# ToyotaResearchInstitute/conex

Measured on AMD Instinct MI355X. Metric: Newton KKT-solves/sec (assemble+factor+solve), 1000x(20x20) PSD blocks, fp64, higher is better.
Workload: dtype f64

## Files before the change

### conex_amd/csrc/dense_elim.hip.h

```cpp
#pragma once
#include "device_utils.h"

namespace cxk {

__device__ __forceinline__ void SqrtAndInverse(double d, double& root, double& inv) {
  const double r0 = __builtin_amdgcn_rsq(d);
  double g = d * r0, h = 0.5 * r0;
  double e = fma(-h, g, 0.5);
  g = fma(g, e, g);
  h = fma(h, e, h);
  e = fma(-h, g, 0.5);
  g = fma(g, e, g);
  h = fma(h, e, h);
  const double res = fma(-g, g, d);
  root = fma(res, h, g);
  inv = h + h;
}

template <int LEN, int C0, int C1, int BASE>
struct DppColumns {
  static __device__ __forceinline__ void run(double (&a)[LEN], double w, double v) {
    if constexpr (C0 < C1) {
      asm("v_fmac_f64_dpp %0, %1, %2 row_newbcast:%3 row_mask:0xf bank_mask:0xf"
          : "+v"(a[C0])
          : "v"(w), "v"(v), "n"(C0 - BASE));
      DppColumns<LEN, C0 + 1, C1, BASE>::run(a, w, v);
    }
  }
};

__device__ __forceinline__ void DppOperandFence(double& x, double& y, double& z) {
  asm("s_nop 1" : "+v"(x), "+v"(y), "+v"(z));
}

__device__ __forceinline__ double EvenRowsToOddRows(double v) {
  typedef unsigned u2 __attribute__((ext_vector_type(2)));
  const unsigned lo = __double2loint(v), hi = __double2hiint(v);
  const u2 a = __builtin_amdgcn_permlane16_swap(lo, lo, false, false);
  const u2 b = __builtin_amdgcn_permlane16_swap(hi, hi, false, false);
  return __hiloint2double(b.x, a.x);
}

template <int NSMAX, int SMAX, int J, int NRHS = 1, bool CHECK = true>
struct ElimSteps {
  static constexpr int LEN = NSMAX + SMAX + NRHS, RB = NSMAX + SMAX;
  static __device__ __forceinline__ void run(double (&a)[LEN], int lane, bool& bad, int ns) {
    if constexpr (J == 0 && NSMAX > 0) {
      const double d = ReadLane(a[0], 0);
      if constexpr (CHECK) bad |= !(d > 0.0);
      double root, inv;
      SqrtAndInverse(d, root, inv);
      step(a, lane, bad, root, inv, ns);
    }
  }
  static __device__ __forceinline__ void step(double (&a)[LEN], int lane, bool& bad, double root, double inv, int ns) {
    if constexpr (J < NSMAX) {
      if (J >= ns) return;
      a[J] = (lane == J) ? root : a[J] * inv;
      double root1 = 1.0, inv1 = 1.0;
      auto next_pivot = [&]() {
        if constexpr (J + 1 < NSMAX) {
          const double d1 = ReadLane(a[J + 1], J + 1);
          if constexpr (CHECK) bad |= !(d1 > 0.0);
          SqrtAndInverse(d1, root1, inv1);
        }
      };
      if constexpr (NSMAX + SMAX <= 16) {
        double naj = -a[J];
        double dummy = 0.0;
        DppOperandFence(dummy, naj, a[J]);
        DppColumns<LEN, J + 1, (J + 2 < NSMAX + SMAX ? J + 2 : NSMAX + SMAX), 0>::run(a, a[J], naj);
        next_pivot();
        DppColumns<LEN, J + 2, NSMAX + SMAX, 0>::run(a, a[J], naj);
      } else if constexpr (NSMAX + SMAX <= 32 && NSMAX != 16) {
        const RowPair xp = Swap16(a[J]);
        double x0 = xp.a, x1 = xp.b;
        double naj = -a[J];
        DppOperandFence(x0, x1, naj);
        constexpr int kEnd = NSMAX + SMAX;
        constexpr int n1 = (J + 2 < kEnd) ? J + 2 : kEnd;
        if constexpr (J + 1 < 16)
          DppColumns<LEN, J + 1, (n1 < 16 ? n1 : 16), 0>::run(a, x0, naj);
        else
          DppColumns<LEN, J + 1, n1, 16>::run(a, x1, naj);
        next_pivot();
        constexpr int kLo0 = (J + 2 < 16) ? J + 2 : 16, kLo1 = (kEnd < 16) ? kEnd : 16;
        constexpr int kHi0 = (J + 2 > 16) ? J + 2 : 16;
        DppColumns<LEN, kLo0, kLo1, 0>::run(a, x0, naj);
        DppColumns<LEN, kHi0, kEnd, 16>::run(a, x1, naj);
      } else if constexpr (NSMAX == 16 && SMAX <= 16) {
        double x = EvenRowsToOddRows(a[J]);
        double naj = -a[J];
        DppOperandFence(x, naj, a[J]);
        DppColumns<LEN, J + 1, (J + 2 < NSMAX ? J + 2 : NSMAX), 0>::run(a, x, naj);
        next_pivot();
        DppColumns<LEN, J + 2, NSMAX, 0>::run(a, x, naj);
        DppColumns<LEN, NSMAX, NSMAX + SMAX, NSMAX>::run(a, a[J], naj);
      } else {
        if constexpr (J + 1 < NSMAX + SMAX) a[J + 1] = fma(-ReadLane(a[J], J + 1), a[J], a[J + 1]);
        next_pivot();
#pragma unroll
        for (int c = J + 2; c < NSMAX + SMAX; c++) a[c] = fma(-ReadLane(a[J], c), a[J], a[c]);
      }
#pragma unroll
      for (int q = 0; q < NRHS; q++) {
        const double yj = ReadLane(a[RB + q], J) * inv;
        if (lane > J)
          a[RB + q] = fma(-yj, a[J], a[RB + q]);
        else if (lane == J)
          a[RB + q] = yj;
      }
      ElimSteps<NSMAX, SMAX, J + 1, NRHS, CHECK>::step(a, lane, bad, root1, inv1, ns);
    }
  }
};

}
```

### conex_amd/csrc/kkt_context.hip

```cpp
#include "kkt_launch.h"
#include "kernels_gemm.hip.h"

namespace cxk_host {

int Fail(cxk_context* ctx, const char* msg) {
  ctx->err = msg;
  fprintf(stderr, "conex_kkt_hip: %s\n", msg);
  return CXK_FAILURE;
}

bool IsUnique(int N, int m, const int* x) {
  std::vector<char> seen(N > 0 ? N : 1, 0);
  for (int i = 0; i < m; i++) {
    if (x[i] >= N || x[i] < 0) return false;
    if (seen[x[i]]++) return false;
  }
  return true;
}

int AddConstraint(cxk_context* ctx, ConstraintRec&& rec, const int* vars) {
  if (!ctx || ctx->finalized) return -1;
  if (vars) {
    if (!IsUnique(ctx->num_vars, rec.m, vars)) return -1;
  } else if (rec.m != ctx->num_vars) {
// ... 1063 lines not shown
  const int n = reps > 0 ? reps : 1;
  for (int r = 0; r < n; r++) {
    CXK_TRY(hipMemcpy(dC.p, C, sizeof(double) * nc * batch, hipMemcpyHostToDevice));
    CXK_TRY(hipEventRecord(e0, nullptr));
    CXK_TRY(LaunchGemmSplitK(g, ta != 0, tb != 0, batch, dP.p, nullptr));
    CXK_TRY(hipEventRecord(e1, nullptr));
    CXK_TRY(hipEventSynchronize(e1));
    float ms = 0;
    CXK_TRY(hipEventElapsedTime(&ms, e0, e1));
    if (r > 0 || n == 1) total += ms;
  }
  if (avg_ms) *avg_ms = total / (n > 1 ? n - 1 : 1);
  CXK_TRY(hipMemcpy(C, dC.p, sizeof(double) * nc * batch, hipMemcpyDeviceToHost));
  (void)hipEventDestroy(e0);
  (void)hipEventDestroy(e1);
  return CXK_SUCCESS;
}

int cxk_dense_top_columns(const cxk_context* ctx) {
  if (!ctx || !ctx->finalized) return -1;
  return ctx->top_dense.on ? ctx->top_dense.args.T : 0;
}

int cxk_count_sparse_lmi(const cxk_context* ctx) {
  if (!ctx || !ctx->finalized) return -1;
  int k = 0;
  for (size_t i = 0; i < ctx->cons.size(); i++) k += ctx->cons[i].type == CXK_LMI && ctx->owned[i] && ctx->cons[i].sparse;
  return k;
}

int cxk_fused_assembly(const cxk_context* ctx) { return ctx && ctx->fused_asm ? 1 : 0; }
int cxk_fused_tree(const cxk_context* ctx) { return ctx && ctx->fused_tree ? 1 : 0; }

int cxk_fused_tree_timed_out(cxk_context* ctx) {
  if (!ctx || !ctx->timeout_unreported) return 0;
  ctx->timeout_unreported = false;
  return 1;
}

int cxk_debug_force_fused_timeout(cxk_context* ctx) {
  if (!ctx || !ctx->fx_flag || !ctx->fused_tree) return CXK_FAILURE;
  *ctx->fx_flag = 1.0;
  return CXK_SUCCESS;
}

int cxk_debug_fused_timeout_at(cxk_context* ctx, int launch_index, int which) {
  if (!ctx || !ctx->device_ready || !ctx->fx_flag || !ctx->fused_tree) return CXK_FAILURE;
  const bool stream_ordered = (which & CXK_DEBUG_FUSED_STREAM_ORDERED) != 0;
  which &= ~CXK_DEBUG_FUSED_STREAM_ORDERED;
  if (stream_ordered && which != CXK_DEBUG_FUSED_SHARD_TOP) return CXK_FAILURE;
  if (which != CXK_DEBUG_FUSED_FACTOR && which != CXK_DEBUG_FUSED_SHARD_UP && which != CXK_DEBUG_FUSED_SHARD_TOP)
    return CXK_FAILURE;
  if ((which == CXK_DEBUG_FUSED_FACTOR) != (ctx->world <= 1) || (ctx->world > 1 && !ctx->fused_shard))
    return CXK_FAILURE;
  ctx->debug_timeout_at = launch_index >= 0 ? ctx->fused_launches + launch_index : -1;
  ctx->debug_timeout_site = which;
  ctx->debug_stream_ordered = stream_ordered;
  return CXK_SUCCESS;
}

int cxk_count_lmi_kernel(const cxk_context* ctx, int which) {
  if (!ctx || !ctx->device_ready) return -1;
  int k = 0;
  for (const Group& g : ctx->groups) {
    if (g.type != CXK_LMI) continue;
    const int kind = g.sparse ? 4 : g.schur_gemm ? 3 : g.mfma ? 2 : 0;
// ... 111 lines not shown
```

### conex_amd/csrc/kkt_plans.hip

```cpp
#include "kkt_internal.h"
#include "big_chol.h"

namespace cxk_host {

void ComputeTreeStructure(cxk_context* ctx) {
  const Layout& L = ctx->lay;
  const int K = ctx->md.K;
  ctx->t_ns.assign(K, 0);
  ctx->t_nsep.assign(K, 0);
  ctx->t_start.assign(K, 0);
  ctx->t_level.assign(K, 0);
  ctx->t_parent.assign(K, -1);
  for (int e = 0; e < K; e++) {
    ctx->t_ns[e] = L.supernode_size[e];
    ctx->t_nsep[e] = (int)L.separators[e].size();
    ctx->t_start[e] = L.supernode_start[e];
    if (ctx->t_nsep[e] > 0) ctx->t_parent[e] = L.var_to_sn[L.separators[e][0]];
  }
  for (int i = 0; i < K; i++) {
    if (ctx->t_ns[i] == 0) continue;
    for (int v : L.separators[i]) {
      const int p = L.var_to_sn[v];
      if (ctx->t_level[p] < ctx->t_level[i] + 1) ctx->t_level[p] = ctx->t_level[i] + 1;
    }
// ... 92 lines not shown
      ctx->sn_mine[e] = 1;
      ctx->owned[i] = (rr++ % G) == ctx->rank;
    } else {
      const bool mine = owner_of_root[root_of[e]] == ctx->rank;
      ctx->sn_mine[e] = mine;
      ctx->owned[i] = mine;
    }
  }
  for (int p = 0; p < ctx->md.N; p++) ctx->var_valid[p] = ctx->sn_mine[ctx->lay.var_to_sn[p]];
  for (int e = 0; e < K; e++)
    if (ctx->sn_top[e]) {
      const int64_t n = ctx->t_ns[e];
      ctx->n_xs += n * (n + 1) / 2 + n * ctx->t_nsep[e];
      ctx->n_xv += (int)n;
    }
}

namespace {

struct PlanSwitches {
  bool no_big_dataflow = getenv("CXK_NO_BIG_DATAFLOW") != nullptr;
  bool debug_levels = getenv("CXK_DEBUG_LEVELS") != nullptr;
  bool no_lean = getenv("CXK_NO_LEAN") != nullptr;
  bool no_ranges = getenv("CXK_NO_RANGES") != nullptr;
  bool keep_top = getenv("CXK_KEEP_TOP") != nullptr;
  bool no_chain = getenv("CXK_NO_CHAIN") != nullptr;
  bool no_back_pairs = getenv("CXK_NO_BACK_PAIRS") != nullptr;
  bool no_fused_asm = getenv("CXK_NO_FUSED_ASM") != nullptr;
  bool no_fused_shard = getenv("CXK_NO_FUSED_SHARD") != nullptr;
  bool no_fused_tree = getenv("CXK_NO_FUSED_TREE") != nullptr;
  bool no_fused_wide = getenv("CXK_NO_FUSED_WIDE") != nullptr;
  bool fused_split = getenv("CXK_FUSED_SPLIT") != nullptr;
  bool fused_level_order = getenv("CXK_FUSED_LEVEL_ORDER") != nullptr;
  bool no_fused_sweep = getenv("CXK_NO_FUSED_SWEEP") != nullptr;
  bool no_top_dense = getenv("CXK_NO_TOP_DENSE") != nullptr;
};

struct Verdict {
  bool ok = true;
  const char* why = nullptr;
  bool check(bool cond, const char* msg) {
    ok = ok && cond;
    if (!ok && !why) why = msg;
    return ok;
  }
  void note(const char* msg) { check(true, msg); }
  int refuse(const PlanSwitches& sw, const char* strategy) const {
    if (sw.debug_levels) fprintf(stderr, "%s not taken: %s\n", strategy, why ? why : "(unnamed check)");
    return CXK_SUCCESS;
  }
};

template <typename Rec>
std::vector<Rec> Flatten(const std::vector<std::vector<int64_t>>& lists, std::vector<int>* ptr, std::vector<int64_t>* src) {
  std::vector<Rec> recs(lists.size());
  ptr->assign(lists.size() + 1, 0);
  for (size_t t = 0; t < lists.size(); t++) {
    for (int64_t q : lists[t]) src->push_back(q);
    (*ptr)[t + 1] = (int)src->size();
    const int len = (*ptr)[t + 1] - (*ptr)[t];
    recs[t].first = len > 0 ? (*src)[(*ptr)[t]] : -1;
    recs[t].beg = (*ptr)[t] + 1;
    recs[t].extra = len > 0 ? len - 1 : 0;
  }
  return recs;
}
// ... 699 lines not shown
  v.check(ok, "a level-0 supernode that is not a leaf with single sources in its own constraint's block");
  if (!v.ok) return v.refuse(sw, "fused assembly");
  std::vector<GatherRec> g2;
  for (size_t t = 0; t < ag.rec.size(); t++)
    if (!slab_own[t]) g2.push_back(ag.rec[t]);
  std::vector<ResidRec> r2;
  std::vector<int> v2;
  for (int pvar = 0; pvar < N; pvar++)
    if (!var_own[pvar]) {
      r2.push_back(rg.rec[pvar]);
      v2.push_back(pvar);
    }
  ctx->as_T2 = (int64_t)g2.size();
  ctx->rs_N2 = (int)v2.size();
  if (g2.empty()) g2.push_back(GatherRec{0, -1, 0, 0});
  if (v2.empty()) {
    r2.push_back(ResidRec{-1, 0, 0});
    v2.push_back(0);
  }
  CXK_TRY(ctx->asm_rec.upload(arecs));
  CXK_TRY(ctx->as_rec2.upload(g2));
  CXK_TRY(ctx->rs_rec2.upload(r2));
  CXK_TRY(ctx->rs_var2.upload(v2));
  ctx->fused_asm = true;
  return CXK_SUCCESS;
}


struct FusedTables {
  std::vector<int> recs, xreg, pub;
  std::vector<long long> xsrc, rsrc;
};

bool FusedTreeShapes(const cxk_context* ctx, const PlanSwitches& sw, const UpdateSlots& u, Verdict& v, int* sa, int* sb) {
  const int nlev = ctx->nlev;
  const std::vector<int>& ns = ctx->t_ns;
  const int cnt_all = (int)ctx->level_sn.size();
  const bool wide_single = v.ok && ctx->world <= 1 && cnt_all == 1 && ctx->md.K >= 1 && ns[ctx->level_sn[0]] > 32 &&
                           ns[ctx->level_sn[0]] <= 64 && ctx->t_nsep[ctx->level_sn[0]] == 0 && !sw.no_fused_wide;
  if (wide_single) {
    *sa = *sb = ((ns[ctx->level_sn[0]] + 7) / 8 * 8) << 8;
    return true;
  }
  std::vector<int> shapes;
  for (int l = 0; l < nlev && v.ok; l++) {
    if (ctx->level_ptr[l + 1] == ctx->level_ptr[l]) continue;
    v.ok = !ctx->level_big[l] && ctx->level_nh[l] == ctx->level_ptr[l + 1] - ctx->level_ptr[l];
    for (auto& sg : ctx->level_segs[l]) {
      v.ok = v.ok && sg.shape != 0 && sg.inl;
      if (std::find(shapes.begin(), shapes.end(), sg.shape) == shapes.end()) shapes.push_back(sg.shape);
    }
    for (int pos = ctx->level_ptr[l]; pos < ctx->level_ptr[l + 1] && v.ok; pos++) {
      const int e = ctx->level_sn[pos];
      v.ok = u.tg_ptr[e + 1] - u.tg_ptr[e] <= kFastTargets && u.m[e] <= kFusedMaxSlots && u.mf[e] <= kFusedMaxSlots;
    }
  }
  for (size_t i = 0; i < shapes.size(); i++)
    if ((shapes[i] & 255) == 0)
      for (size_t j = 0; j < shapes.size(); j++)
        if (j != i && shapes[i] >= 0 && (shapes[j] >> 8) == (shapes[i] >> 8) && (shapes[j] & 255) > 0) {
          shapes[i] = -1;
          break;
        }
  shapes.erase(std::remove(shapes.begin(), shapes.end(), -1), shapes.end());
  std::sort(shapes.begin(), shapes.end());
  v.note("a level without a register shape, inline separator lists or within the slot limits");
  v.check(!shapes.empty() && shapes.size() <= 2, "more than two register shapes");
  if (v.ok) {
    *sa = shapes[0];
    *sb = shapes.back();
  }
  return false;
}

void FusedTreeRecords(const cxk_context* ctx, const AsmGather& ag, const ResidGather& rg, const ExchangeLayout& x,
                      int cnt_up, int wide_shape, Verdict& v, FusedTables* ft) {
  const MatrixData& md = ctx->md;
  const Layout& L = ctx->lay;
  const std::vector<int>& ns = ctx->t_ns;
  const std::vector<int>& start = ctx->t_start;
  const int cnt_all = (int)ctx->level_sn.size();
  std::vector<int>& recs = ft->recs;
  recs.assign((size_t)cnt_all * kFusedRecWords, 0);
  for (int pos = 0; pos < cnt_all && v.ok; pos++) {
    const int e = ctx->level_sn[pos];
    const int i = md.clique_order[e];
    const int m = ctx->cons[i].m;
    const IntList& r = md.supernodes_pos[e];
    const IntList& sp = md.separators_pos[e];
    const int nse = (int)r.size(), nsp = (int)sp.size();
    const int nsm = wide_shape ? wide_shape >> 8 : RegisterShape(ns[e], ctx->t_nsep[e]) >> 8;
    int* w = recs.data() + (size_t)pos * kFusedRecWords;
    if (pos >= cnt_up) {
      if (!v.check(ctx->sn_top[e] && nsm > 0 && x.xs_base[e] >= 0 && ctx->n_xs < (int64_t)INT32_MAX,
                   "a top supernode without a register kernel"))
        break;
      memcpy(w, &ctx->h_recs[pos], sizeof(SnRec));
      w[32] = (int)(x.xs_base[e] & 0xffffffffll);
      w[33] = (int)(x.xs_base[e] >> 32);
      w[34] = x.xv_base[e];
      w[63] = ctx->t_level[e];
      continue;
    }
// ... 502 lines not shown
```

### conex_amd/csrc/tree_fused.h

```cpp
#pragma once
#include <hip/hip_runtime.h>

#include <cstdint>

namespace cxk {

constexpr unsigned long long kFusedSentinel = 0x7FF4C0DEC0DE5EEDull;

constexpr int kFusedRecWords = 64;
constexpr int kFusedExtraTargets = 128;
constexpr int kFusedExtraSlots = 8;
constexpr int kFusedExtraMax = 64;
constexpr int kFusedMaxSlots = 4096;

struct GatherRec;
struct ResidRec;

struct FusedTreeArgs {
  const int* rec;
  int count;
  const double *G, *AWc, *AQcc, *b;
  double *AW, *AQc;
  double* slab;
  double* y;
// ... 10 lines not shown
  int gen;
  int tgen;
  long long fwd_stride, y_stride;
  double* y3;
  int* fail;
  int tag;
  double k, bs, cs;
  double cb, cq, cw;
  int comb;
  int form;
  const double* k_from;
  const double* sc;
  double* sys_sc;
  int K;
  double* host_flag;
  int up_sleep;
  int count_up;
  double* x;
  long long n_xs;
  int n_xv;
  const GatherRec* xg;
  const int64_t* as_src;
  const int* xs_pt;
  const int* pt_ptr;
  const int64_t* pt_src;
  const ResidRec* xr;
  const int64_t* rs_src;
  const int* pf_ptr;
  const int* pf_src;
  unsigned long long* done;
  unsigned long long done_target;
};

constexpr int FusedRhsLane(int nsmax, int smax) { return (nsmax == 16 && smax == 8) || (nsmax == 24 && smax == 0) ? 24 : -1; }

enum FusedTreeMode { kFusedFull = 0, kFusedSolve = 1, kFusedUp = 2, kFusedForward = 3, kFusedDown = 4,
                     kFusedShardUp = 5, kFusedShardTop = 6, kFusedTriple = 7 };

bool FusedTreeCompiled(int shape_a, int shape_b);
int FusedTreeOccupancy(int shape_a, int shape_b, bool sharded = false);
hipError_t LaunchFusedTree(const FusedTreeArgs& a, int shape_a, int shape_b, int mode, hipStream_t stream,
                           hipEvent_t ev_start = nullptr, hipEvent_t ev_stop = nullptr);

}
```

### conex_amd/csrc/tree_fused.hip

```cpp
#include <hip/hip_runtime.h>
#include <hip/hip_ext.h>

#include <type_traits>

#include "tree_supernode.hip.h"
#include "kernels_kkt_top.hip.h"
#include "tree_fused.h"

namespace cxk {

constexpr int kFusedSpinLimit = 1 << 18;

#ifdef CXK_FUSED_STAMPS
constexpr int kFusedStampWaves = 8192;
__device__ long long g_fused_tree_stamp[kFusedStampWaves * 16];
#define FT_STAMP(i) ft_stamp[i] = __builtin_amdgcn_s_memrealtime()
#define FT_COUNT(i, v) ft_stamp[i] = (v)
#define FT_STAMP_DECL long long ft_stamp[16] = {0, 0, 0, 0, 0, 0, 0, 0, 0, 0, 0, 0, 0, 0, 0, 0}
#define FT_STAMP_FLUSH(level)                                                              \
  do {                                                                                     \
    if ((threadIdx.x & 63) == 0 && blockIdx.x < kFusedStampWaves) {                        \
      ft_stamp[15] = (level);                                                              \
      for (int i_ = 0; i_ < 16; i_++) g_fused_tree_stamp[blockIdx.x * 16 + i_] = ft_stamp[i_]; \
    }                                                                                      \
// ... 542 lines not shown
#pragma unroll
  for (int qq = 0; qq < (QN > 0 ? QN : 1); qq++) {
    yv[qq] = 0.0;
#pragma unroll
    for (int q = 0; q < (NRHS > 1 ? NRHS - 1 : 1); q++) yvx[q][qq] = 0.0;
  }
  if constexpr (QN > 0) {
#pragma unroll
    for (int qq = 0; qq < QN; qq++) {
      const unsigned sw = qq < cnt ? (unsigned)R.sep[qq] : 0u;
      bv[qq] = my[65 * li + NSMAX + (int)(sw >> 26)];
    }
  }
#pragma unroll
  for (int k = 0; k < NSMAX; k++) col[k] = (active && k > lane && k < ns) ? col[k] : 0.0;
  dg = active ? dg : 1.0;
  double ub, ubx[NRHS > 1 ? NRHS - 1 : 1];
  ubx[0] = 0.0;
  if constexpr (ROWRHS) {
    ub = active ? my[65 * li + RL] : 0.0;
#pragma unroll
    for (int q = 0; q < NRHS - 1; q++) ubx[q] = active ? my[65 * li + RL + 1 + q] : 0.0;
  } else {
    ub = active ? a[NCOL > 0 ? RB : 0] : 0.0;
#pragma unroll
    for (int q = 0; q < NCOL - 1; q++) ubx[q] = active ? a[RB + 1 + q] : 0.0;
  }
  if constexpr (QN > 0) {
#pragma unroll
    for (int qq = 0; qq < QN; qq++) Mb[qq] = (qq < cnt && active) ? bv[qq] : 0.0;
  }
  {
    const double dinv = 1.0 / dg;
#pragma unroll
    for (int k = NSMAX - 1; k >= 0; k--) {
      if (lane == k) ub *= dinv;
      ub = fma(-col[k], ReadLane(ub, k), ub);
      if constexpr (NRHS > 1) {
#pragma unroll
        for (int q = 0; q < NRHS - 1; q++) {
          if (lane == k) ubx[q] *= dinv;
          ubx[q] = fma(-col[k], ReadLane(ubx[q], k), ubx[q]);
        }
      }
      if constexpr (QN > 0) {
        if (cnt > 0) {
#pragma unroll
          for (int qq = 0; qq < QN; qq++) {
            if (lane == k) Mb[qq] *= dinv;
            Mb[qq] = fma(-col[k], ReadLane(Mb[qq], k), Mb[qq]);
          }
        }
      }
    }
  }
  constexpr bool ROW0 = NSMAX <= 16 && QN > 0;
  double vsep = 0.0, vsepx[NRHS > 1 ? NRHS - 1 : 1];
#pragma unroll
  for (int q = 0; q < (NRHS > 1 ? NRHS - 1 : 1); q++) vsepx[q] = 0.0;
  if constexpr (ROW0) {
#pragma unroll
    for (int qq = 0; qq < QN; qq++) {
      Mb[qq] = -Mb[qq];
      asm volatile("" : "+v"(Mb[qq]));
    }
  }
  if constexpr (QN > 0) {
    if (cnt > 0) {
      const int sepw = __builtin_amdgcn_ds_bpermute(4 * (24 + (lane < 8 ? lane : 0)), w);
      const int sidx = lane < cnt ? (sepw & 0x3ffffff) : (R.sep[0] & 0x3ffffff);
      const double* src = ysG + sidx;
      double v;
      double vx[NRHS > 1 ? NRHS - 1 : 1];
      vx[0] = 0.0;
      for (int spin = 0;; spin++) {
        v = LoadAgent(src);
        bool pending = (lane < cnt) & IsSentinel(v);
        if constexpr (NRHS > 1) {
#pragma unroll
          for (int q = 0; q < NRHS - 1; q++) {
            vx[q] = LoadAgent(ysT + (int64_t)(1 + q) * A.y_stride + sidx);
            pending |= (lane < cnt) & IsSentinel(vx[q]);
// ... 265 lines not shown
  }
  if constexpr (SMAX > 0 && PHASE != 2) {
    if (s > 0) {
#pragma unroll
      for (int r = 0; r < PR; r++) {
        const int t = lane + 64 * r;
        const int d = A.pub[pub_beg + (t < nv ? t : 0)];
        if (t < nv) StoreAgent(handO + d, SentinelValue());
      }
    }
  }
}

__device__ __forceinline__ void FusedScalars(const FusedTreeArgs& A) {
  const int lane = threadIdx.x & 63;
  double t0 = 0, t1 = 0;
#pragma unroll
  for (int v = 0; v < 4; v++) {
    double s0 = 0, s1 = 0;
    for (int i = 64 * v + lane; i < A.K; i += 256) {
      s0 += A.sc[2 * i];
      s1 += A.sc[2 * i + 1];
    }
    t0 += WaveSum(s0);
    t1 += WaveSum(s1);
  }
  if (lane == 0) {
    A.sys_sc[0] = t0;
    A.sys_sc[1] = t1;
    *A.fail = 0;
  }
}

template <int NA, int SA, int NB, int SB, int MODE>
__global__ void __launch_bounds__(64, 2) tree_fused(FusedTreeArgs A) {
  extern __shared__ double lds[];
  const int pos = blockIdx.x;
  if (pos >= A.count) {
    FusedScalars(A);
    return;
  }
  const int w = A.rec[(size_t)pos * kFusedRecWords + (threadIdx.x & 63)];
  const int ns = __builtin_amdgcn_readlane(w, 1), s = __builtin_amdgcn_readlane(w, 2);
  constexpr int NRHS = MODE == 2 ? 3 : 1;
  if (NA == NB && SA == SB) {
    FusedSupernode<NA, SA, MODE == 1, false, NRHS>(A, w, lds);
  } else if (RegisterShape(ns, s) == (NA << 8 | SA)) {
    FusedSupernode<NA, SA, MODE == 1, false, NRHS>(A, w, lds);
  } else {
    FusedSupernode<NB, SB, MODE == 1, false, NRHS>(A, w, lds);
  }
}

__device__ __forceinline__ double WaitValue(const FusedTreeArgs& A, const double* p) {
  double v = LoadAgent(p);
  for (int spin = 0; IsSentinel(v); spin++) {
    if (spin >= kFusedSpinLimit) {
      atomicExch(A.fail + 1, A.tag);
      __hip_atomic_store(A.host_flag, 1.0, __ATOMIC_RELAXED, __HIP_MEMORY_SCOPE_SYSTEM);
      break;
    }
    __builtin_amdgcn_s_sleep(1);
    v = LoadAgent(p);
  }
  return v;
}

__device__ __forceinline__ void ShardPackItem(const FusedTreeArgs& A, int64_t item) {
  const double* handG = A.hand + (int64_t)A.gen * A.hand_stride;
  if (item < A.n_xs) {
    const GatherRec g = A.xg[item];
    double s = 0;
    if (g.first >= 0) s += A.G[g.first];
    for (int k = g.beg; k < g.beg + g.extra; k++) {
      const int64_t q = A.as_src[k];
      if (q >= 0) s += A.G[q];
    }
    const int t = A.xs_pt[item];
    if (t >= 0) {
      double u = 0;
// ... 31 lines not shown
      const unsigned long long have = __hip_atomic_load(A.done + 16 * lane, __ATOMIC_RELAXED, __HIP_MEMORY_SCOPE_AGENT);
      if (__ballot(have < want) == 0) break;
      if (spin >= kFusedSpinLimit) {
        if (lane == 0) {
          atomicExch(A.fail + 1, A.tag);
          __hip_atomic_store(A.host_flag, 1.0, __ATOMIC_RELAXED, __HIP_MEMORY_SCOPE_SYSTEM);
        }
        break;
      }
      __builtin_amdgcn_s_sleep(2);
    }
  }
  if (lane == 0) {
    const int64_t o = A.n_xs + 3 * (int64_t)A.n_xv;
    const int f0 = __hip_atomic_load(A.fail, __ATOMIC_RELAXED, __HIP_MEMORY_SCOPE_AGENT);
    const int f1 = __hip_atomic_load(A.fail + 1, __ATOMIC_RELAXED, __HIP_MEMORY_SCOPE_AGENT);
    A.x[o] = A.sys_sc[0];
    A.x[o + 1] = A.sys_sc[1];
    const bool tagged = A.tag != 0 && f1 == A.tag;
    A.x[o + 2] = (f0 != 0 || tagged) ? 1.0 : 0.0;
    A.x[o + 3] = tagged && __hip_atomic_load(A.host_flag, __ATOMIC_RELAXED, __HIP_MEMORY_SCOPE_SYSTEM) != 0.0 ? 1.0 : 0.0;
  }
}

template <int NA, int SA, int NB, int SB>
__global__ void __launch_bounds__(64) tree_fused_shard_up(FusedTreeArgs A) {
  extern __shared__ double lds[];
  const int pos = blockIdx.x;
  if (pos < A.count_up) {
    const int w = A.rec[(size_t)pos * kFusedRecWords + (threadIdx.x & 63)];
    const int ns = __builtin_amdgcn_readlane(w, 1), s = __builtin_amdgcn_readlane(w, 2);
    if (NA == NB && SA == SB) {
      FusedSupernode<NA, SA, true>(A, w, lds);
    } else if (RegisterShape(ns, s) == (NA << 8 | SA)) {
      FusedSupernode<NA, SA, true>(A, w, lds);
    } else {
      FusedSupernode<NB, SB, true>(A, w, lds);
    }
    if ((threadIdx.x & 63) == 0) {
      __builtin_amdgcn_fence(__ATOMIC_RELEASE, "workgroup");
      __hip_atomic_fetch_add(A.done + 16 * (pos & 63), 1ull, __ATOMIC_RELAXED, __HIP_MEMORY_SCOPE_AGENT);
    }
    return;
  }
  const int64_t items = A.n_xs + A.n_xv;
  const int64_t first = (int64_t)(pos - A.count_up) * 64;
  if (first < items) {
    ShardPackItem(A, first + (threadIdx.x & 63));
    return;
  }
  ShardPackTail(A);
}

template <int NA, int SA, int NB, int SB>
__global__ void __launch_bounds__(64) tree_fused_shard_top(FusedTreeArgs A) {
  extern __shared__ double lds[];
  const int b = blockIdx.x, ntop = A.count - A.count_up;
  if (b >= A.count) {
    if ((threadIdx.x & 63) == 0) {
      const int64_t o = A.n_xs + 3 * (int64_t)A.n_xv;
      A.sys_sc[0] = A.x[o];
      A.sys_sc[1] = A.x[o + 1];
      if (A.x[o + 2] > 0.0) *A.fail = 1;
    }
    return;
  }
  const int pos = b < ntop ? A.count_up + b : A.count - 1 - b;
  const int w = A.rec[(size_t)pos * kFusedRecWords + (threadIdx.x & 63)];
  const int ns = __builtin_amdgcn_readlane(w, 1), s = __builtin_amdgcn_readlane(w, 2);
  const bool isA = (NA == NB && SA == SB) || RegisterShape(ns, s) == (NA << 8 | SA);
  if (b < ntop) {
    if (isA)
      FusedSupernode<NA, SA, false, true>(A, w, lds);
    else
      FusedSupernode<NB, SB, false, true>(A, w, lds);
  } else {
    if (isA)
      FusedSolveSupernode<NA, SA, 2>(A, w);
    else
      FusedSolveSupernode<NB, SB, 2>(A, w);
  }
}

template <int NA, int SA, int NB, int SB, int PHASE>
__global__ void __launch_bounds__(64) tree_fused_solve(FusedTreeArgs A) {
  const int pos = PHASE == 2 ? A.count - 1 - (int)blockIdx.x : (int)blockIdx.x;
  const int w = A.rec[(size_t)pos * kFusedRecWords + (threadIdx.x & 63)];
  const int ns = __builtin_amdgcn_readlane(w, 1), s = __builtin_amdgcn_readlane(w, 2);
  if (NA == NB && SA == SB) {
    FusedSolveSupernode<NA, SA, PHASE>(A, w);
  } else if (RegisterShape(ns, s) == (NA << 8 | SA)) {
    FusedSolveSupernode<NA, SA, PHASE>(A, w);
  } else {
    FusedSolveSupernode<NB, SB, PHASE>(A, w);
  }
}

namespace {
constexpr int FusedImage(int nsmax, int smax) { return 65 * nsmax > 64 * (smax + 3) ? 65 * nsmax : 64 * (smax + 3); }

struct FusedKernels {
  const void* k[8];
  int image;
};

template <int NA, int SA, int NB, int SB>
FusedKernels KernelsOf() {
  FusedKernels f;
  f.k[kFusedFull] = reinterpret_cast<const void*>(&tree_fused<NA, SA, NB, SB, 0>);
  f.k[kFusedSolve] = reinterpret_cast<const void*>(&tree_fused_solve<NA, SA, NB, SB, 0>);
  f.k[kFusedUp] = reinterpret_cast<const void*>(&tree_fused<NA, SA, NB, SB, 1>);
  f.k[kFusedForward] = reinterpret_cast<const void*>(&tree_fused_solve<NA, SA, NB, SB, 1>);
  f.k[kFusedDown] = reinterpret_cast<const void*>(&tree_fused_solve<NA, SA, NB, SB, 2>);
  f.k[kFusedShardUp] = nullptr;
  f.k[kFusedShardTop] = nullptr;
  f.k[kFusedTriple] = nullptr;
  if constexpr (NA <= 32 && NB <= 32) f.k[kFusedTriple] = reinterpret_cast<const void*>(&tree_fused<NA, SA, NB, SB, 2>);
  if constexpr (NA <= 32 && NB <= 32) {
    f.k[kFusedShardUp] = reinterpret_cast<const void*>(&tree_fused_shard_up<NA, SA, NB, SB>);
    f.k[kFusedShardTop] = reinterpret_cast<const void*>(&tree_fused_shard_top<NA, SA, NB, SB>);
  }
  f.image = FusedImage(NA, SA) > FusedImage(NB, SB) ? FusedImage(NA, SA) : FusedImage(NB, SB);
  return f;
}

bool ForPair(int sa, int sb, FusedKernels* out) {
#define CXK_FUSED_PAIR(NA_, SA_, NB_, SB_)                          \
  if (sa == ((NA_) << 8 | (SA_)) && sb == ((NB_) << 8 | (SB_))) {   \
    if (out) *out = KernelsOf<NA_, SA_, NB_, SB_>();                \
    return true;                                                    \
  }
  CXK_FUSED_PAIR(8, 8, 8, 8)
  CXK_FUSED_PAIR(16, 8, 16, 8)
  CXK_FUSED_PAIR(24, 0, 24, 0)
  CXK_FUSED_PAIR(24, 8, 24, 8)
  CXK_FUSED_PAIR(32, 16, 32, 16)
  CXK_FUSED_PAIR(8, 8, 16, 8)
  CXK_FUSED_PAIR(8, 8, 24, 0)
  CXK_FUSED_PAIR(8, 8, 24, 8)
  CXK_FUSED_PAIR(8, 8, 32, 16)
  CXK_FUSED_PAIR(16, 8, 24, 0)
  CXK_FUSED_PAIR(16, 8, 24, 8)
  CXK_FUSED_PAIR(16, 8, 32, 16)
  CXK_FUSED_PAIR(24, 0, 24, 8)
  CXK_FUSED_PAIR(24, 0, 32, 16)
  CXK_FUSED_PAIR(24, 8, 32, 16)
  CXK_FUSED_PAIR(40, 0, 40, 0)
  CXK_FUSED_PAIR(48, 0, 48, 0)
  CXK_FUSED_PAIR(56, 0, 56, 0)
  CXK_FUSED_PAIR(64, 0, 64, 0)
#undef CXK_FUSED_PAIR
  return false;
}
}

bool FusedTreeCompiled(int sa, int sb) { return ForPair(sa, sb, nullptr); }

int FusedTreeOccupancy(int sa, int sb, bool sharded) {
  FusedKernels f;
  if (!ForPair(sa, sb, &f)) return 0;
  int nb = 0, nbs = 0;
  if (sharded) {
    if (!f.k[kFusedShardTop]) return 0;
    if (hipOccupancyMaxActiveBlocksPerMultiprocessor(&nb, f.k[kFusedShardTop], 64, sizeof(double) * (size_t)f.image) != hipSuccess) return 0;
    return nb;
  }
  if (hipOccupancyMaxActiveBlocksPerMultiprocessor(&nb, f.k[kFusedFull], 64, sizeof(double) * (size_t)f.image) != hipSuccess) return 0;
  if (hipOccupancyMaxActiveBlocksPerMultiprocessor(&nbs, f.k[kFusedSolve], 64, 0) != hipSuccess) return 0;
  return nb < nbs ? nb : nbs;
}

hipError_t LaunchFusedTree(const FusedTreeArgs& a, int sa, int sb, int mode, hipStream_t stream, hipEvent_t ev_start,
                           hipEvent_t ev_stop) {
  FusedKernels f;
// ... 21 lines not shown
```

### conex_amd/kkt.py

```python
import ctypes as C
import os

import numpy as np

LIB_PATH = os.path.join(os.path.dirname(os.path.abspath(__file__)), "lib", "libconex.so")
_LIB = None

c_int_p = C.POINTER(C.c_int)
c_long_p = C.POINTER(C.c_long)
c_double_p = C.POINTER(C.c_double)


def _dp(a):
    return a.ctypes.data_as(c_double_p)


def _ip(a):
    return a.ctypes.data_as(c_int_p)


def _lp(a):
    return a.ctypes.data_as(c_long_p)


# ... 602 lines not shown
        self._check(self.L.cxk_exchange_download(self.h, _dp(out)), "cxk_exchange_download")
        return out

    def exchange_upload(self, x):
        x = np.ascontiguousarray(x, dtype=np.float64)
        self._check(self.L.cxk_exchange_upload(self.h, _dp(x)), "cxk_exchange_upload")

    def exchange_tensor(self, torch):
        ptr, count = self.exchange_buffer()

        class _Arr:
            __cuda_array_interface__ = {"shape": (count,), "typestr": "<f8", "data": (ptr, False),
                                        "version": 2}
        return torch.as_tensor(_Arr(), device="cuda")

    def assemble_local(self):
        self._check(self.L.cxk_assemble_local(self.h), "cxk_assemble_local")

    def finish_assemble(self):
        self._check(self.L.cxk_finish_assemble(self.h), "cxk_finish_assemble")

    def dense_top_columns(self):
        return self.L.cxk_dense_top_columns(self.h)

    def count_sparse_lmi(self):
        return self.L.cxk_count_sparse_lmi(self.h)

    def fused_assembly(self):
        return bool(self.L.cxk_fused_assembly(self.h))

    def fused_tree(self):
        return bool(self.L.cxk_fused_tree(self.h))

    def count_lmi_kernel(self, which):
        return self.L.cxk_count_lmi_kernel(self.h, which)

    def lmi_kernels(self, i):
        out = (C.c_int * 5)()
        self._check(self.L.cxk_lmi_kernels(self.h, i, out), "cxk_lmi_kernels")
        return {s: self.L.cxk_lmi_kernel_name(out[j]).decode() for j, s in enumerate(LMI_STAGES)}

    def step_info(self):
        out = np.zeros(2 * self.K)
        self._check(self.L.cxk_get_step_info(self.h, _dp(out)), "cxk_get_step_info")
        return out.reshape(self.K, 2)

    def assembly_work(self):
        b = C.c_double()
        f = C.c_double()
        self.L.cxk_assembly_work(self.h, C.byref(b), C.byref(f))
        return b.value, f.value

    def enable_timing(self, on=True):
        self.L.cxk_enable_timing(self.h, int(on))

    def kernel_time(self, reset=True):
        ms = C.c_double()
        n = self.L.cxk_kernel_time(self.h, int(reset), C.byref(ms))
        return n, ms.value

    CLOCKS = {"assembly": 0, "tree": 1, "solve": 2, "query": 3, "prepare": 4, "take": 5}

    def kernel_clock(self, which, reset=True):
        ms = C.c_double()
        n = self.L.cxk_kernel_clock(self.h, self.CLOCKS[which] if isinstance(which, str) else int(which),
                                    int(reset), C.byref(ms))
# ... 54 lines not shown
```

### include/conex_kkt_hip.h

```cpp
#ifndef CONEX_KKT_HIP_H
#define CONEX_KKT_HIP_H

#ifdef __cplusplus
extern "C" {
#endif

typedef struct cxk_context cxk_context;

enum { CXK_SUCCESS = 0, CXK_FAILURE = 1 };

enum {
  CXK_LMI = 0,
  CXK_LINEAR = 1,
  CXK_SOC = 2,
  CXK_STATIC = 3,
  CXK_QUAD = 4,
  CXK_OCT = 5
};

int cxk_create(int num_vars, int device, void* stream, cxk_context** out);
void cxk_destroy(cxk_context* ctx);
const char* cxk_last_error(const cxk_context* ctx);

int cxk_add_lmi(cxk_context* ctx, int n, int m, const double* A ,
// ... 111 lines not shown
int cxk_get_valid_variables(const cxk_context* ctx, unsigned char* mask );
int cxk_shard_info(const cxk_context* ctx, int* cut_level, int* num_levels, long* exchange_count);
int cxk_assemble_local(cxk_context* ctx);
int cxk_finish_assemble(cxk_context* ctx);

int cxk_get_step_info(cxk_context* ctx, double* out2k);

int cxk_line_search(cxk_context* ctx, double dinf_upper_bound, double b_scaling, double c_scaling,
                    double* result);

int cxk_gemm_f64(int device, int ta, int tb, int M, int N, int K, int batch, const double* A,
                 const double* B, double* C, double alpha, double beta, int lower_only, int splits,
                 int reps, double* avg_ms);

int cxk_count_sparse_lmi(const cxk_context* ctx);

int cxk_count_lmi_kernel(const cxk_context* ctx, int which);

enum {
  CXK_LMI_STAGE_SCHUR = 0,
  CXK_LMI_STAGE_PREPARE = 1,
  CXK_LMI_STAGE_QUERY = 2,
  CXK_LMI_STAGE_TAKE = 3,
  CXK_LMI_STAGE_AFFINE = 4
};
int cxk_lmi_kernels(const cxk_context* ctx, int constraint, int out[5]);
const char* cxk_lmi_kernel_name(int code);
int cxk_lmi_kernel_count(void);

int cxk_dense_top_columns(const cxk_context* ctx);

int cxk_fused_assembly(const cxk_context* ctx);
int cxk_fused_tree(const cxk_context* ctx);
int cxk_fused_tree_timed_out(cxk_context* ctx);
int cxk_debug_force_fused_timeout(cxk_context* ctx);
enum { CXK_DEBUG_FUSED_FACTOR = 0, CXK_DEBUG_FUSED_SHARD_UP = 1, CXK_DEBUG_FUSED_SHARD_TOP = 2,
       CXK_DEBUG_FUSED_STREAM_ORDERED = 16 };
int cxk_debug_fused_timeout_at(cxk_context* ctx, int launch_index, int which);

int cxk_assembly_work(const cxk_context* ctx, double* bytes, double* flops);
int cxk_kernel_time(cxk_context* ctx, int reset, double* avg_ms);
enum { CXK_CLOCK_ASSEMBLY = 0, CXK_CLOCK_TREE = 1, CXK_CLOCK_SOLVE = 2, CXK_CLOCK_QUERY = 3,
       CXK_CLOCK_PREPARE = 4, CXK_CLOCK_TAKE = 5, CXK_CLOCK_COUNT = 6 };
int cxk_kernel_clock(cxk_context* ctx, int which, int reset, double* avg_ms);
int cxk_set_iterative_refinement(cxk_context* ctx, int iterations);

int cxk_enable_timing(cxk_context* ctx, int on);

#ifdef __cplusplus
}
#endif
#endif
```

Before: 22880.

## Software-pipeline pivot sqrt with DPP eliminations and use tighter fused-tree register frames

Rewrites the 17-32 column dense Cholesky elimination step so the next pivot's broadcast, reciprocal square root and Newton refinement are interleaved with the current column's DPP fmac updates, using sched barriers to pin the order. It also adds tight frame selection, which picks the smallest compiled register shape (new 16x5 / 20x0 pair) that covers all supernodes instead of padded frames, and dispatches by fit rather than exact shape. The aim is to hide pivot-sqrt latency and cut wasted lanes and registers for 20x20 blocks, in exchange for heavier hand-scheduled inline asm and extra kernel instantiations.

```diff
diff --git a/conex_amd/csrc/dense_elim.hip.h b/conex_amd/csrc/dense_elim.hip.h
--- a/conex_amd/csrc/dense_elim.hip.h
+++ b/conex_amd/csrc/dense_elim.hip.h
@@ -33,12 +33,56 @@
   asm("s_nop 1" : "+v"(x), "+v"(y), "+v"(z));
 }
 
-__device__ __forceinline__ double EvenRowsToOddRows(double v) {
+
+template <int NSMAX, int SMAX, int J, int C, int LEN>
+__device__ __forceinline__ void ElimFmac(double (&a)[LEN], double x0, double x1) {
+  if constexpr (C < 16) {
+    asm volatile("v_fmac_f64_dpp %0, %1, -%2 row_newbcast:%3 row_mask:0xf bank_mask:0xf"
+                 : "+v"(a[C])
+                 : "v"(x0), "v"(a[J]), "n"(C));
+  } else if constexpr (NSMAX == 16) {
+    asm volatile("v_fmac_f64_dpp %0, %1, -%1 row_newbcast:%2 row_mask:0xf bank_mask:0xf"
+                 : "+v"(a[C])
+                 : "v"(a[J]), "n"(C - 16));
+  } else {
+    asm volatile("v_fmac_f64_dpp %0, %1, -%2 row_newbcast:%3 row_mask:0xf bank_mask:0xf"
+                 : "+v"(a[C])
+                 : "v"(x1), "v"(a[J]), "n"(C - 16));
+  }
+}
+
+template <int NSMAX, int SMAX, int J, int P0, int CNT, int N, int LEN>
+__device__ __forceinline__ void ElimIssue(double (&a)[LEN], double x0, double x1) {
+  if constexpr (CNT > 0 && P0 < N) {
+    ElimFmac<NSMAX, SMAX, J, J + 1 + P0>(a, x0, x1);
+    ElimIssue<NSMAX, SMAX, J, P0 + 1, CNT - 1, N>(a, x0, x1);
+  }
+}
+
+__device__ __forceinline__ int OpaqueLane(int lane) {
+  int z;
+  asm volatile("s_mov_b32 %0, 0" : "=s"(z));
+  return lane + z;
+}
+
+template <int J>
+__device__ __forceinline__ double ElimPivotColumn(double v, int lz, unsigned long long& m, double& s0, double& s1) {
   typedef unsigned u2 __attribute__((ext_vector_type(2)));
-  const unsigned lo = __double2loint(v), hi = __double2hiint(v);
-  const u2 a = __builtin_amdgcn_permlane16_swap(lo, lo, false, false);
-  const u2 b = __builtin_amdgcn_permlane16_swap(hi, hi, false, false);
-  return __hiloint2double(b.x, a.x);
+  __builtin_amdgcn_sched_barrier(0);
+  m = __builtin_amdgcn_ballot_w64(lz == J);
+  asm volatile("" : : "s"(m));
+  __builtin_amdgcn_sched_barrier(0);
+  double c0, c1;
+  asm volatile("v_mov_b64 %0, %2\n\tv_mov_b64 %1, %2" : "=&v"(c0), "=&v"(c1) : "v"(v));
+  __builtin_amdgcn_sched_barrier(0);
+  const double d = ReadLane(v, J);
+  __builtin_amdgcn_sched_barrier(0);
+  const u2 l = __builtin_amdgcn_permlane16_swap(__double2loint(c0), __double2loint(c1), false, false);
+  const u2 h = __builtin_amdgcn_permlane16_swap(__double2hiint(c0), __double2hiint(c1), false, false);
+  s0 = __hiloint2double(h.x, l.x);
+  s1 = __hiloint2double(h.y, l.y);
+  __builtin_amdgcn_sched_barrier(0);
+  return d;
 }
 
 template <int NSMAX, int SMAX, int J, int NRHS = 1, bool CHECK = true>
@@ -46,15 +90,80 @@
   static constexpr int LEN = NSMAX + SMAX + NRHS, RB = NSMAX + SMAX;
   static __device__ __forceinline__ void run(double (&a)[LEN], int lane, bool& bad, int ns) {
     if constexpr (J == 0 && NSMAX > 0) {
-      const double d = ReadLane(a[0], 0);
-      if constexpr (CHECK) bad |= !(d > 0.0);
-      double root, inv;
-      SqrtAndInverse(d, root, inv);
-      step(a, lane, bad, root, inv, ns);
+      if constexpr (kPipelined) {
+        unsigned long long m;
+        double s0, s1;
+        const int lz = OpaqueLane(lane);
+        const double d = ElimPivotColumn<0>(a[0], lz, m, s0, s1);
+        if constexpr (CHECK) bad |= !(d > 0.0);
+        double root, inv;
+        SqrtAndInverse(d, root, inv);
+        step(a, lane, bad, root, inv, ns, lz, m, s0, s1);
+      } else {
+        const double d = ReadLane(a[0], 0);
+        if constexpr (CHECK) bad |= !(d > 0.0);
+        double root, inv;
+        SqrtAndInverse(d, root, inv);
+        step(a, lane, bad, root, inv, ns);
+      }
     }
   }
-  static __device__ __forceinline__ void step(double (&a)[LEN], int lane, bool& bad, double root, double inv, int ns) {
-    if constexpr (J < NSMAX) {
+  static constexpr bool kPipelined = NSMAX + SMAX > 16 && NSMAX + SMAX <= 32;
+  static __device__ __forceinline__ void step(double (&a)[LEN], int lane, bool& bad, double root, double inv, int ns,
+                                              int lz = 0, unsigned long long m = 0, double s0 = 0.0, double s1 = 0.0) {
+    if constexpr (kPipelined && J < NSMAX) {
+      if (J >= ns) return;
+      constexpr int N = NSMAX + SMAX - J - 1;
+      const double x0 = s0 * inv, x1 = s1 * inv, t = a[J] * inv;
+      __builtin_amdgcn_sched_barrier(0);
+      a[J] = __builtin_amdgcn_inverse_ballot_w64(m) ? root : t;
+      __builtin_amdgcn_sched_barrier(0);
+      if constexpr (NSMAX == 16 && J + 1 >= 16 && N > 0) asm volatile("s_nop 1");
+      ElimIssue<NSMAX, SMAX, J, 0, 1, N>(a, x0, x1);
+      double root1 = 1.0, inv1 = 1.0, t0 = 0.0, t1 = 0.0;
+      unsigned long long m1 = 0;
+      if constexpr (J + 1 < NSMAX) {
+        const double d1 = ElimPivotColumn<J + 1>(a[J + 1], lz, m1, t0, t1);
+        if constexpr (CHECK) bad |= !(d1 > 0.0);
+#define CXK_ELIM_FILL(P0, CNT)                      \
+  __builtin_amdgcn_sched_barrier(0);                \
+  ElimIssue<NSMAX, SMAX, J, P0, CNT, N>(a, x0, x1); \
+  __builtin_amdgcn_sched_barrier(0)
+        const double r0 = __builtin_amdgcn_rsq(d1);
+        CXK_ELIM_FILL(1, 2);
+        double g = d1 * r0, hh = 0.5 * r0;
+        CXK_ELIM_FILL(3, 2);
+        double e = fma(-hh, g, 0.5);
+        CXK_ELIM_FILL(5, 2);
+        g = fma(g, e, g);
+        hh = fma(hh, e, hh);
+        CXK_ELIM_FILL(7, 2);
+        e = fma(-hh, g, 0.5);
+        CXK_ELIM_FILL(9, 2);
+        g = fma(g, e, g);
+        hh = fma(hh, e, hh);
+        CXK_ELIM_FILL(11, 2);
+        const double res = fma(-g, g, d1);
+        inv1 = hh + hh;
+        CXK_ELIM_FILL(13, 2);
+        root1 = fma(res, hh, g);
+        CXK_ELIM_FILL(15, 64);
+#undef CXK_ELIM_FILL
+        asm volatile("" : : "v"(root1), "v"(inv1));
+      } else {
+        ElimIssue<NSMAX, SMAX, J, 1, 64, N>(a, x0, x1);
+        __builtin_amdgcn_sched_barrier(0);
+      }
+#pragma unroll
+      for (int q = 0; q < NRHS; q++) {
+        const double yj = ReadLane(a[RB + q], J) * inv;
+        if (lane > J)
+          a[RB + q] = fma(-yj, a[J], a[RB + q]);
+        else if (lane == J)
+          a[RB + q] = yj;
+      }
+      ElimSteps<NSMAX, SMAX, J + 1, NRHS, CHECK>::step(a, lane, bad, root1, inv1, ns, lz, m1, t0, t1);
+    } else if constexpr (J < NSMAX) {
       if (J >= ns) return;
       a[J] = (lane == J) ? root : a[J] * inv;
       double root1 = 1.0, inv1 = 1.0;
@@ -72,30 +181,6 @@
         DppColumns<LEN, J + 1, (J + 2 < NSMAX + SMAX ? J + 2 : NSMAX + SMAX), 0>::run(a, a[J], naj);
         next_pivot();
         DppColumns<LEN, J + 2, NSMAX + SMAX, 0>::run(a, a[J], naj);
-      } else if constexpr (NSMAX + SMAX <= 32 && NSMAX != 16) {
-        const RowPair xp = Swap16(a[J]);
-        double x0 = xp.a, x1 = xp.b;
-        double naj = -a[J];
-        DppOperandFence(x0, x1, naj);
-        constexpr int kEnd = NSMAX + SMAX;
-        constexpr int n1 = (J + 2 < kEnd) ? J + 2 : kEnd;
-        if constexpr (J + 1 < 16)
-          DppColumns<LEN, J + 1, (n1 < 16 ? n1 : 16), 0>::run(a, x0, naj);
-        else
-          DppColumns<LEN, J + 1, n1, 16>::run(a, x1, naj);
-        next_pivot();
-        constexpr int kLo0 = (J + 2 < 16) ? J + 2 : 16, kLo1 = (kEnd < 16) ? kEnd : 16;
-        constexpr int kHi0 = (J + 2 > 16) ? J + 2 : 16;
-        DppColumns<LEN, kLo0, kLo1, 0>::run(a, x0, naj);
-        DppColumns<LEN, kHi0, kEnd, 16>::run(a, x1, naj);
-      } else if constexpr (NSMAX == 16 && SMAX <= 16) {
-        double x = EvenRowsToOddRows(a[J]);
-        double naj = -a[J];
-        DppOperandFence(x, naj, a[J]);
-        DppColumns<LEN, J + 1, (J + 2 < NSMAX ? J + 2 : NSMAX), 0>::run(a, x, naj);
-        next_pivot();
-        DppColumns<LEN, J + 2, NSMAX, 0>::run(a, x, naj);
-        DppColumns<LEN, NSMAX, NSMAX + SMAX, NSMAX>::run(a, a[J], naj);
       } else {
         if constexpr (J + 1 < NSMAX + SMAX) a[J + 1] = fma(-ReadLane(a[J], J + 1), a[J], a[J + 1]);
         next_pivot();
diff --git a/conex_amd/csrc/kkt_context.hip b/conex_amd/csrc/kkt_context.hip
--- a/conex_amd/csrc/kkt_context.hip
+++ b/conex_amd/csrc/kkt_context.hip
@@ -1119,6 +1119,13 @@
 int cxk_fused_assembly(const cxk_context* ctx) { return ctx && ctx->fused_asm ? 1 : 0; }
 int cxk_fused_tree(const cxk_context* ctx) { return ctx && ctx->fused_tree ? 1 : 0; }
 
+int cxk_fused_tree_frames(const cxk_context* ctx, int* frame_a, int* frame_b) {
+  if (!ctx || !frame_a || !frame_b) return CXK_FAILURE;
+  *frame_a = ctx->fused_tree ? ctx->fused_sa : 0;
+  *frame_b = ctx->fused_tree ? ctx->fused_sb : 0;
+  return CXK_SUCCESS;
+}
+
 int cxk_fused_tree_timed_out(cxk_context* ctx) {
   if (!ctx || !ctx->timeout_unreported) return 0;
   ctx->timeout_unreported = false;
diff --git a/conex_amd/csrc/kkt_plans.hip b/conex_amd/csrc/kkt_plans.hip
--- a/conex_amd/csrc/kkt_plans.hip
+++ b/conex_amd/csrc/kkt_plans.hip
@@ -148,6 +148,7 @@
   bool no_fused_wide = getenv("CXK_NO_FUSED_WIDE") != nullptr;
   bool fused_split = getenv("CXK_FUSED_SPLIT") != nullptr;
   bool fused_level_order = getenv("CXK_FUSED_LEVEL_ORDER") != nullptr;
+  bool fused_padded_frames = getenv("CXK_FUSED_PADDED_FRAMES") != nullptr;
   bool no_fused_sweep = getenv("CXK_NO_FUSED_SWEEP") != nullptr;
   bool no_top_dense = getenv("CXK_NO_TOP_DENSE") != nullptr;
 };
@@ -913,6 +914,32 @@
   std::vector<long long> xsrc, rsrc;
 };
 
+void TightFrames(const cxk_context* ctx, int* sa, int* sb) {
+  const int pa = *sa, pb = *sb;
+  int mn[2] = {0, 0}, ms[2] = {0, 0};
+  for (int e : ctx->level_sn) {
+    const int n = ctx->t_ns[e], s = ctx->t_nsep[e];
+    const int g = (pa == pb || (n <= (pa >> 8) && s <= (pa & 255))) ? 0 : 1;
+    mn[g] = std::max(mn[g], n);
+    ms[g] = std::max(ms[g], s);
+  }
+  int tight[2] = {pa, pb};
+  for (int g = 0; g < 2; g++) {
+    const int padded = g == 0 ? pa : pb;
+    for (int f : kFusedFrames)
+      if (mn[g] <= (f >> 8) && ms[g] <= (f & 255) && (f >> 8) <= (padded >> 8) && (f & 255) <= (padded & 255) &&
+          (ms[g] == 0 || (f >> 8) == (padded >> 8))) {
+        tight[g] = f;
+        break;
+      }
+  }
+  if (pa == pb) tight[1] = tight[0];
+  if (tight[0] <= tight[1] && FusedTreeCompiled(tight[0], tight[1])) {
+    *sa = tight[0];
+    *sb = tight[1];
+  }
+}
+
 bool FusedTreeShapes(const cxk_context* ctx, const PlanSwitches& sw, const UpdateSlots& u, Verdict& v, int* sa, int* sb) {
   const int nlev = ctx->nlev;
   const std::vector<int>& ns = ctx->t_ns;
@@ -950,6 +977,7 @@
   if (v.ok) {
     *sa = shapes[0];
     *sb = shapes.back();
+    if (!sw.fused_padded_frames && ctx->world <= 1) TightFrames(ctx, sa, sb);
   }
   return false;
 }
diff --git a/conex_amd/csrc/tree_fused.h b/conex_amd/csrc/tree_fused.h
--- a/conex_amd/csrc/tree_fused.h
+++ b/conex_amd/csrc/tree_fused.h
@@ -66,12 +66,15 @@
   unsigned long long done_target;
 };
 
-constexpr int FusedRhsLane(int nsmax, int smax) { return (nsmax == 16 && smax == 8) || (nsmax == 24 && smax == 0) ? 24 : -1; }
+constexpr int FusedRhsLane(int nsmax, int smax) {
+  return (nsmax == 16 && (smax == 8 || smax == 5)) || ((nsmax == 24 || nsmax == 20) && smax == 0) ? 24 : -1;
+}
 
 enum FusedTreeMode { kFusedFull = 0, kFusedSolve = 1, kFusedUp = 2, kFusedForward = 3, kFusedDown = 4,
                      kFusedShardUp = 5, kFusedShardTop = 6, kFusedTriple = 7 };
 
 bool FusedTreeCompiled(int shape_a, int shape_b);
+constexpr int kFusedFrames[] = {8 << 8 | 8, 16 << 8 | 5, 16 << 8 | 8, 20 << 8 | 0, 24 << 8 | 0, 24 << 8 | 8, 32 << 8 | 16};
 int FusedTreeOccupancy(int shape_a, int shape_b, bool sharded = false);
 hipError_t LaunchFusedTree(const FusedTreeArgs& a, int shape_a, int shape_b, int mode, hipStream_t stream,
                            hipEvent_t ev_start = nullptr, hipEvent_t ev_stop = nullptr);
diff --git a/conex_amd/csrc/tree_fused.hip b/conex_amd/csrc/tree_fused.hip
--- a/conex_amd/csrc/tree_fused.hip
+++ b/conex_amd/csrc/tree_fused.hip
@@ -598,14 +598,15 @@
   }
   {
     const double dinv = 1.0 / dg;
+    const int lzb = OpaqueLane(lane);
 #pragma unroll
     for (int k = NSMAX - 1; k >= 0; k--) {
-      if (lane == k) ub *= dinv;
+      if (lzb == k) ub *= dinv;
       ub = fma(-col[k], ReadLane(ub, k), ub);
       if constexpr (NRHS > 1) {
 #pragma unroll
         for (int q = 0; q < NRHS - 1; q++) {
-          if (lane == k) ubx[q] *= dinv;
+          if (lzb == k) ubx[q] *= dinv;
           ubx[q] = fma(-col[k], ReadLane(ubx[q], k), ubx[q]);
         }
       }
@@ -613,7 +614,7 @@
         if (cnt > 0) {
 #pragma unroll
           for (int qq = 0; qq < QN; qq++) {
-            if (lane == k) Mb[qq] *= dinv;
+            if (lzb == k) Mb[qq] *= dinv;
             Mb[qq] = fma(-col[k], ReadLane(Mb[qq], k), Mb[qq]);
           }
         }
@@ -945,6 +946,9 @@
   }
 }
 
+template <int NA, int SA>
+__device__ __forceinline__ bool FitsFrame(int ns, int s) { return ns <= NA && s <= SA; }
+
 template <int NA, int SA, int NB, int SB, int MODE>
 __global__ void __launch_bounds__(64, 2) tree_fused(FusedTreeArgs A) {
   extern __shared__ double lds[];
@@ -958,7 +962,7 @@
   constexpr int NRHS = MODE == 2 ? 3 : 1;
   if (NA == NB && SA == SB) {
     FusedSupernode<NA, SA, MODE == 1, false, NRHS>(A, w, lds);
-  } else if (RegisterShape(ns, s) == (NA << 8 | SA)) {
+  } else if (FitsFrame<NA, SA>(ns, s)) {
     FusedSupernode<NA, SA, MODE == 1, false, NRHS>(A, w, lds);
   } else {
     FusedSupernode<NB, SB, MODE == 1, false, NRHS>(A, w, lds);
@@ -1056,7 +1060,7 @@
     const int ns = __builtin_amdgcn_readlane(w, 1), s = __builtin_amdgcn_readlane(w, 2);
     if (NA == NB && SA == SB) {
       FusedSupernode<NA, SA, true>(A, w, lds);
-    } else if (RegisterShape(ns, s) == (NA << 8 | SA)) {
+    } else if (FitsFrame<NA, SA>(ns, s)) {
       FusedSupernode<NA, SA, true>(A, w, lds);
     } else {
       FusedSupernode<NB, SB, true>(A, w, lds);
@@ -1092,7 +1096,7 @@
   const int pos = b < ntop ? A.count_up + b : A.count - 1 - b;
   const int w = A.rec[(size_t)pos * kFusedRecWords + (threadIdx.x & 63)];
   const int ns = __builtin_amdgcn_readlane(w, 1), s = __builtin_amdgcn_readlane(w, 2);
-  const bool isA = (NA == NB && SA == SB) || RegisterShape(ns, s) == (NA << 8 | SA);
+  const bool isA = (NA == NB && SA == SB) || FitsFrame<NA, SA>(ns, s);
   if (b < ntop) {
     if (isA)
       FusedSupernode<NA, SA, false, true>(A, w, lds);
@@ -1113,7 +1117,7 @@
   const int ns = __builtin_amdgcn_readlane(w, 1), s = __builtin_amdgcn_readlane(w, 2);
   if (NA == NB && SA == SB) {
     FusedSolveSupernode<NA, SA, PHASE>(A, w);
-  } else if (RegisterShape(ns, s) == (NA << 8 | SA)) {
+  } else if (FitsFrame<NA, SA>(ns, s)) {
     FusedSolveSupernode<NA, SA, PHASE>(A, w);
   } else {
     FusedSolveSupernode<NB, SB, PHASE>(A, w);
@@ -1128,7 +1132,7 @@
   int image;
 };
 
-template <int NA, int SA, int NB, int SB>
+template <int NA, int SA, int NB, int SB, bool SHARDED = true>
 FusedKernels KernelsOf() {
   FusedKernels f;
   f.k[kFusedFull] = reinterpret_cast<const void*>(&tree_fused<NA, SA, NB, SB, 0>);
@@ -1140,7 +1144,7 @@
   f.k[kFusedShardTop] = nullptr;
   f.k[kFusedTriple] = nullptr;
   if constexpr (NA <= 32 && NB <= 32) f.k[kFusedTriple] = reinterpret_cast<const void*>(&tree_fused<NA, SA, NB, SB, 2>);
-  if constexpr (NA <= 32 && NB <= 32) {
+  if constexpr (SHARDED && NA <= 32 && NB <= 32) {
     f.k[kFusedShardUp] = reinterpret_cast<const void*>(&tree_fused_shard_up<NA, SA, NB, SB>);
     f.k[kFusedShardTop] = reinterpret_cast<const void*>(&tree_fused_shard_top<NA, SA, NB, SB>);
   }
@@ -1164,6 +1168,10 @@
   CXK_FUSED_PAIR(8, 8, 24, 8)
   CXK_FUSED_PAIR(8, 8, 32, 16)
   CXK_FUSED_PAIR(16, 8, 24, 0)
+  if (sa == (16 << 8 | 5) && sb == (20 << 8 | 0)) {
+    if (out) *out = KernelsOf<16, 5, 20, 0, false>();
+    return true;
+  }
   CXK_FUSED_PAIR(16, 8, 24, 8)
   CXK_FUSED_PAIR(16, 8, 32, 16)
   CXK_FUSED_PAIR(24, 0, 24, 8)
diff --git a/conex_amd/kkt.py b/conex_amd/kkt.py
--- a/conex_amd/kkt.py
+++ b/conex_amd/kkt.py
@@ -658,6 +658,13 @@
     def fused_tree(self):
         return bool(self.L.cxk_fused_tree(self.h))
 
+    def fused_tree_frames(self):
+        fn = self.L.cxk_fused_tree_frames
+        fn.restype, fn.argtypes = C.c_int, [C.c_void_p, C.POINTER(C.c_int), C.POINTER(C.c_int)]
+        a, b = C.c_int(0), C.c_int(0)
+        self._check(fn(self.h, C.byref(a), C.byref(b)), "cxk_fused_tree_frames")
+        return (a.value >> 8, a.value & 255), (b.value >> 8, b.value & 255)
+
     def count_lmi_kernel(self, which):
         return self.L.cxk_count_lmi_kernel(self.h, which)
 
diff --git a/include/conex_kkt_hip.h b/include/conex_kkt_hip.h
--- a/include/conex_kkt_hip.h
+++ b/include/conex_kkt_hip.h
@@ -167,6 +167,7 @@
 
 int cxk_fused_assembly(const cxk_context* ctx);
 int cxk_fused_tree(const cxk_context* ctx);
+int cxk_fused_tree_frames(const cxk_context* ctx, int* frame_a, int* frame_b);
 int cxk_fused_tree_timed_out(cxk_context* ctx);
 int cxk_debug_force_fused_timeout(cxk_context* ctx);
 enum { CXK_DEBUG_FUSED_FACTOR = 0, CXK_DEBUG_FUSED_SHARD_UP = 1, CXK_DEBUG_FUSED_SHARD_TOP = 2,
```

New measurement: 24280, median of 6. 6.1% higher.
